# CodeKnight314/Goal-Conditioned-RL-Framework

Measured on AMD Instinct MI355X. Metric: gradient-steps/sec (HER sample + critic+actor update), higher is better.
Workload: dtype f32; 1 GPU; ddpg_pickplace_b256; agent=DDPG, batch_per_gpu=256, buffer_rows=1000000, state_dim=23, action_dim=4, hidden=256, layers=3, k_future=8, gradient_step=40, parallelism=single, hip_graph=True, rng=cpython-mt19937 (host) indices

## Files before the change

goal-conditioned-rl-framework_amd/csrc/agent.hip:

```cpp
#include <hip/hip_runtime.h>

#include <algorithm>
#include <cmath>
#include <cstdlib>
#include <map>
#include <mutex>
#include <random>
#include <string>
#include <vector>

#include "act_bn.h"
#include "dw_adam.h"
#include "gemm_mfma.h"
#include "her_ring.h"
#include "meet.h"
#include "ops.h"
#include "rowchain.h"
#include "sac_heads.h"
#include "xchg_ipc.h"
#include "pop.h"
#include "pbt_host.h"

using namespace gcrl;

// ... 40 lines not shown
  StepCtrl more[kMaxStepsPerCall - 1];
};

}

struct StepPlan { int variant; int tuple_len; };
struct DpSeg { int kind, a, b; float* reduce; long long reduce_n; };

struct gcrl_agent {
  gcrl_agent_config cfg;
  int S = 0, A = 0, H = 0, L = 0, B = 0, C = 0, ldx = 0, Mmax = 0, Apad = 0;
  int Q = 1;
  bool has_target_actor = false, sac = false;
  NetSpec actor, critic;
  hipStream_t stream = nullptr, cap_stream = nullptr;

  float *params = nullptr, *grads = nullptr, *adam_m = nullptr, *adam_v = nullptr;
  long long n_params = 0, n_grads = 0;
  long long off_actor = 0, off_tactor = 0, off_critic = 0, off_tcritic = 0, off_logalpha = 0;
  long long goff_critic = 0, goff_actor = 0, goff_alpha = 0;
  long long critic_stride = 0;
  float *bn_rmean = nullptr, *bn_rvar = nullptr;
  float* alpha_dev = nullptr;

  float* work = nullptr;
  float *sa = nullptr, *nsa = nullptr, *spa = nullptr, *rbuf = nullptr, *dbuf = nullptr;
  long long slot_x = 0, slot_rd = 0;
  float *hTA[2] = {}, *hA = nullptr, *hC = nullptr, *hTC = nullptr, *gC = nullptr, *gA[2] = {};
  float *hC2 = nullptr, *gC2 = nullptr, *bn_part = nullptr;
  float* red_scratch = nullptr;
  float* red_td() const { return red_scratch; }
  float* red_sel() const { return red_scratch + 64LL * ((B + 255) / 256); }
  unsigned int* red_ticket(int i) const { return reinterpret_cast<unsigned int*>(red_scratch + 72LL * ((B + 255) / 256) + 32 * i); }
  float *q = nullptr, *qt = nullptr, *q2 = nullptr, *dq = nullptr, *dq2 = nullptr, *dact = nullptr;
  float *zA = nullptr, *xhatA = nullptr, *invstdA = nullptr, *headA = nullptr, *ghead = nullptr, *dh2 = nullptr;
  float *zN = nullptr, *hN = nullptr, *headN = nullptr, *bn_partN = nullptr;
  float *logp = nullptr, *logp_next = nullptr, *epsbuf = nullptr, *stdbuf = nullptr;
  float *noise_in = nullptr, *eps_next_in = nullptr, *eps_cur_in = nullptr, *norm_partial = nullptr;
  float *w_in = nullptr, *td_abs = nullptr;
  float *act_in = nullptr, *act_tmp[2] = {};
  float *qy = nullptr, *q_row_loss = nullptr, *q_row_td = nullptr;
  float* pi_buf = nullptr;
  float* act_pinned = nullptr;
  char *oa_pinned = nullptr, *oa_dev = nullptr;
  char* act_fl_host = nullptr; char* act_fl_dev = nullptr; unsigned long long act_seq = 0;
  long long oa_calls = 0, oa_launches = 0, oa_copies = 0, oa_syncs = 0;
  size_t oa_bytes = 0;
  bool rowchain = false, wt_dirty = true;
  BnSync bn_sync;
  gcrl_dp* bn_sync_dp = nullptr;
  gcrl_exchange_fn bn_sync_fn = nullptr;
  void* bn_sync_user = nullptr;
  float* bn_sync_buf = nullptr;
  long long bn_sync_cap = 0;
  gcrl_xchg* bn_xchg_h = nullptr;
  int dw_split_c = 1, dw_split_a = 1;
  float *dw_part = nullptr, *dw_tick = nullptr;
  std::vector<long long> dwp_off_c, dwp_off_a, dwt_off_c, dwt_off_a;
  long long dwp_cstride = 0, dwt_cstride = 0, dwp_actor = 0, dwt_actor = 0;
  bool dw_batch_off = false;
  bool bn_slab = false;
  bool slab_on() const { return bn_slab && bn_sync.world <= 1; }
  float* bn_bstat = nullptr;
  float *bn_xchg = nullptr, *bn_bar = nullptr;
  bool bn_split_all = std::getenv("GCRL_NO_SLAB_SPLIT_ALL") == nullptr;
  bool tg_fold_off = std::getenv("GCRL_NO_TG_FOLD") != nullptr;
  bool heads_fold_off = std::getenv("GCRL_NO_HEADS_FOLD") != nullptr;
  const float *hf_eps_next = nullptr, *hf_eps_cur = nullptr;
  int hf_nf = 0;
  int bn_rsplit = 1;
  int bn_slots = 0;
  bool heads_fused_off = false;
  bool red_off = false;
  bool layer_adv_off = false;
  bool bn_fused_tiled = true;
  bool bn_fused = false;
  bool split_k = false;
  bool split_roles = false;
  int n_cus = 0;
  bool rc_merge = false;
  bool rc_merge_k = false;
  bool ddpg_ksplit = false, ddpg_ksplit_can = false;
  bool opt_fuse = false, opt_fuse_can = false;
  long long of_wgs = 0;
  float *of_slots = nullptr, *of_seq = nullptr;
  long long of_stride = 0;
  float* rc_bar = nullptr;
  long long rc_bar_words = 0;
  bool rowtile = false, rowtile_can = false;
  float *rt_xb = nullptr, *rt_qpart = nullptr, *rt_ctr = nullptr, *rt_xid = nullptr;
  long long rt_xb_floats = 0, rt_part_floats = 0;
  long long rt_ctr_words = 0;
  unsigned int *status_host = nullptr, *status_dev = nullptr;
  gcrl_xchg* xchg = nullptr;
  bool xchg_sep_norm = false;
  float xchg_scale() const { return xchg ? 1.0f / (float)gcrl_xchg_world(xchg) : 1.0f; }
  int split_rg[4] = {1, 1, 1, 1};
  int row_rg = 1, row_ldl = 0;
  float *wt = nullptr, *rc_gC = nullptr, *rc_gA = nullptr, *ybuf = nullptr;
  long long wt_net[4] = {};
  long long wt_cstride = 0;
  bool prof = false;
  static constexpr int kProfPairs = 64;
  hipEvent_t prof_a[kProfPairs] = {}, prof_b[kProfPairs] = {};
  unsigned long long* prof_clk = nullptr;
  int prof_used = 0;
  int64_t prof_launches = 0;
  double prof_ms = 0, prof_ticks = 0;
  float *parts_c = nullptr, *parts_a = nullptr;
  int nparts_c = 0, nparts_a = 0, part_off_bn = 0;
  std::vector<int> part_off_c, part_off_a;

  char* upload_dev = nullptr;
  size_t upload_bytes = 0;
  char* upload_pinned[kCtrlSlots] = {};
  hipEvent_t upload_ev[kCtrlSlots] = {};
  int next_upload = 0;
  float *metrics_host = nullptr, *metrics_dev = nullptr;
  int64_t next_ticket = 0;
  int64_t fetched_upto = -1;
  std::vector<int> ticket_len;
  hipEvent_t call_ev[kEventRing] = {};
  int64_t call_last_ticket[kEventRing];
  int64_t calls = 0;

  int64_t t_actor = 0, t_critic = 0, t_alpha = 0;
  double lr_actor = 0, lr_critic = 0;
  uint64_t rng_ctr = 0;
  int pending_variant = 0;
  struct { gcrl_her* her = nullptr; int n = 0; int slot = 0; int next = 0; } deferred;
  int head_batches = 2;
  std::vector<StepPlan> dp_plans;
  std::vector<DpSeg> dp_segs;
  size_t dp_pos = 0;

  std::map<int, hipGraphExec_t> graphs;
  std::map<std::string, std::pair<float*, long long>> names;

  hipStream_t pick(void* s) const {
    if (!s) return stream;
    if (s == GCRL_STREAM_LEGACY) return (hipStream_t) nullptr;
    return (hipStream_t)s;
  }
  CtrlBlock* ctrl() const { return (CtrlBlock*)upload_dev; }
  uint32_t* idx_dev() const { return (uint32_t*)(upload_dev + sizeof(UploadBlock)); }
  const StepCtrl* cur() const { return &ctrl()->cur; }
  const StepCtrl* prev() const { return &ctrl()->prev; }
  const int* slot_ptr() const { return &ctrl()->cur.batch_slot; }
  float* P_actor() const { return params + off_actor; }
  float* P_tactor() const { return params + off_tactor; }
  float* P_critic(int c) const { return params + off_critic + c * critic_stride; }
  float* P_tcritic(int c) const { return params + off_tcritic + c * critic_stride; }
  float* P_logalpha() const { return params + off_logalpha; }
  float* G_actor() const { return grads + goff_actor; }
  float* G_critic(int c) const { return grads + goff_critic + c * critic_stride; }
  float* hC_at(int c, int l) const { return hC + ((long long)c * L + l) * B * H; }
  float* hTC_at(int c, int i) const { return hTC + ((long long)c * 2 + i) * B * H; }
  float* gC_at(int c, int i) const { return gC + ((long long)c * 2 + i) * B * H; }
  float* hC2_at(int l) const { return hC2 + (long long)l * B * H; }
  float* gC2_at(int i) const { return gC2 + (long long)i * B * H; }
  float* hA_at(int l) const { return hA + (long long)l * B * H; }
  int n_actor_critics() const { return (cfg.kind == GCRL_AGENT_DDPG || cfg.kind == GCRL_AGENT_TD3) ? 1 : C; }
};

namespace {

// ... 1047 lines not shown
      {&a->q, (long long)C * B * a->Q}, {&a->qt, (long long)C * B * a->Q}, {&a->q2, (long long)C * B * a->Q}, {&a->dq, (long long)C * B * a->Q},
      {&a->dq2, (long long)C * B * a->Q}, {&a->qy, (long long)B * 64}, {&a->q_row_loss, (long long)C * B}, {&a->q_row_td, B}, {&a->dact, (long long)C * B * a->Apad}, {&a->zA, BH}, {&a->xhatA, L * BH},
      {&a->invstdA, (long long)L * H}, {&a->headA, (long long)B * 2 * a->Apad}, {&a->ghead, (long long)B * 2 * a->Apad},
      {&a->dh2, BH}, {&a->logp, B}, {&a->logp_next, B}, {&a->epsbuf, (long long)B * A}, {&a->stdbuf, (long long)B * A},
      {&a->noise_in, (long long)B * A}, {&a->eps_next_in, (long long)B * A}, {&a->eps_cur_in, (long long)B * A},
      {&a->norm_partial, (long long)kMaxCritics * kNormBlocks}, {&a->act_in, (long long)B * a->ldx},
      {&a->act_tmp[0], BH}, {&a->act_tmp[1], BH},
      {&a->parts_c, (long long)C * a->nparts_c}, {&a->parts_a, (long long)a->nparts_a},
      {&a->hC2, (long long)C * L * BH}, {&a->gC2, 2 * BH}, {&a->bn_part, 2LL * ((B + 15) / 16) * H},
      {&a->rc_gC, (long long)C * L * BH}, {&a->rc_gA, L * BH}, {&a->ybuf, B}, {&a->pi_buf, (long long)B * a->Apad},
      {&a->w_in, B}, {&a->td_abs, B}, {&a->red_scratch, 72LL * ((B + 255) / 256) + 64},
      {&a->bn_bstat, 2LL * 2 * L * H}, {&a->bn_xchg, bn_slab_xchg_floats(H)}, {&a->bn_bar, bn_slab_bar_words(H)}, {&a->zN, BH}, {&a->hN, 2 * BH}, {&a->headN, (long long)B * 2 * a->Apad}, {&a->bn_partN, 2LL * ((B + 15) / 16) * H}};
  {
    const long long per_a = (long long)round_up(S, 4) * H + (long long)(L - 1) * H * H;
    const long long per_c = (long long)a->ldx * H + (long long)(L - 1) * H * H;
    a->wt_cstride = align_up(per_c, 64);
    a->wt_net[0] = 0; a->wt_net[1] = align_up(per_a, 64);
    a->wt_net[2] = 2 * align_up(per_a, 64); a->wt_net[3] = a->wt_net[2] + C * a->wt_cstride;
    wants.push_back({&a->wt, a->wt_net[3] + C * a->wt_cstride});
    a->row_ldl = round_up(std::max(H, a->ldx), 4) + 4;
    a->row_rg = row_rg_of(c.kind, B);
    a->rowchain = (c.kind == GCRL_AGENT_DDPG || c.kind == GCRL_AGENT_TD3 || c.kind == GCRL_AGENT_SAC) && H % 4 == 0 &&
                  c.pipeline_steps >= 2 &&
                  rowchain_lds_bytes(a->row_rg, a->row_ldl, A, H, C) <= 160 * 1024;
    a->split_roles = a->rowchain && c.kind == GCRL_AGENT_SAC && sac_split_roles_rule(C, B, a->row_rg);
    for (int i = 0; i < 4; ++i) a->split_rg[i] = a->row_rg;
    {
      const long long nblk = (B + 4 * a->row_rg - 1) / (4 * a->row_rg);
      a->rc_merge = a->split_roles && !std::getenv("GCRL_NO_RC_MERGE") && !std::getenv("GCRL_SPLIT_RG") &&
                    rowchain_merge_ok(a->row_rg, a->row_ldl, A, H, C, B);
      if (a->rc_merge) { a->rc_bar_words = 2 * nblk * 32; wants.push_back({&a->rc_bar, a->rc_bar_words}); }
    }
    a->split_k = a->rowchain && c.kind == GCRL_AGENT_TD3 && C == 2 && td3_split_k_rule(B, a->row_rg);
    a->rc_merge_k = a->split_k && !meet_device_shared() && !std::getenv("GCRL_NO_RC_MERGE");
    if (a->rc_merge_k && !a->rc_bar_words) {
      const long long nblk = (B + 4 * a->row_rg - 1) / (4 * a->row_rg);
      a->rc_bar_words = 2 * nblk * 32;
      wants.push_back({&a->rc_bar, a->rc_bar_words});
    }
    a->rowtile_can = a->rowchain && c.kind == GCRL_AGENT_DDPG && C == 1 && rowtile_shape_ok(B, H, L, S, A, C);
    a->rowtile = a->rowtile_can && rowtile_enabled() && rowtile_ok(B, H, L, S, A, C);
    if (a->rowtile_can) {
      a->rt_ctr_words = rowtile_ctr_words(B, L);
      a->rt_xb_floats = rowtile_xb_floats(B, H, L); a->rt_part_floats = rowtile_part_floats(B, H);
      wants.push_back({&a->rt_xb, a->rt_xb_floats});
      wants.push_back({&a->rt_qpart, a->rt_part_floats}); wants.push_back({&a->rt_ctr, 2 * a->rt_ctr_words});
      wants.push_back({&a->rt_xid, 3LL * (B / 16) * 32});
    }
    {
      const long long nblk = (B + 4 * a->row_rg - 1) / (4 * a->row_rg);
      static const int per_cu = std::getenv("GCRL_DDPG_KSPLIT_PER_CU") ? std::atoi(std::getenv("GCRL_DDPG_KSPLIT_PER_CU")) : 1;
      a->ddpg_ksplit_can = a->rowchain && c.kind == GCRL_AGENT_DDPG && C == 1 && 3 * nblk <= per_cu * std::max(a->n_cus, 1);
      a->ddpg_ksplit = a->ddpg_ksplit_can && !meet_device_shared() && !std::getenv("GCRL_NO_DDPG_KSPLIT");
      if (a->ddpg_ksplit_can && !a->rc_bar_words) { a->rc_bar_words = 2 * nblk * 32; wants.push_back({&a->rc_bar, a->rc_bar_words}); }
    }
    {
      auto tiles16 = [&](const NetSpec& net, bool* form1) {
        long long t = 0;
        for (const Lin& ln : net.lin) {
          GemmDesc d = bwd_dw(a->grads, 1, a->grads, 1, a->grads, ln, B);
          if (gemm_shape_of(d) != 1) *form1 = false;
          t += (long long)((ln.out + 15) / 16) * ((ln.in + 1 + 15) / 16);
        }
        return t;
      };
      bool form1 = true;
      const long long tc = tiles16(a->critic, &form1), ta = tiles16(a->actor, &form1);
      const long long cap = dw_adam_capacity();
      a->of_stride = align_up(std::max(tc, ta) + 8, 32);
      const bool kind_ok = (c.kind == GCRL_AGENT_DDPG && C == 1) || ((c.kind == GCRL_AGENT_TD3 || c.kind == GCRL_AGENT_SAC) && C == 2);
      a->opt_fuse_can = a->rowchain && kind_ok && L + 1 <= kFusedMaxLayers && form1 && B < 2048 &&
                        std::max(tc, ta) <= 256LL * kFusedMaxSlotsPerThread && 2 * std::max(tc, ta) <= cap;
      a->opt_fuse = a->opt_fuse_can && !meet_device_shared() && !std::getenv("GCRL_NO_OPT_FUSE");
      a->of_wgs = 2 * std::max(tc, ta);
      if (a->opt_fuse_can) {
        wants.push_back({&a->of_slots, (long long)(C + 1) * 2 * a->of_stride * 2});
        wants.push_back({&a->of_seq, (long long)(C + 1) * 32});
      }
    }
    a->head_batches = 3;
    if (c.kind == GCRL_AGENT_DDPG && c.pipeline_steps != 0) a->head_batches = 4;
    if (const char* e = std::getenv("GCRL_HEAD_BATCHES")) a->head_batches = std::max(1, std::min(8, std::atoi(e)));
    a->dw_batch_off = std::getenv("GCRL_NO_DW_BATCH") != nullptr;
    a->bn_fused_tiled = std::getenv("GCRL_NO_BN_TILED_STATS") == nullptr;
    a->layer_adv_off = std::getenv("GCRL_NO_LAYER_ADV") != nullptr;
    a->red_off = std::getenv("GCRL_NO_MB_REDUCE") != nullptr;
    a->heads_fused_off = std::getenv("GCRL_NO_HEADS_FUSED") != nullptr;
    a->bn_fused = std::getenv("GCRL_BN_FUSED") != nullptr;
    if (const char* e = std::getenv("GCRL_SPLIT_RG"))
      for (int i = 0; i < 4 && e[i]; ++i) a->split_rg[i] = e[i] - '0';
  }
  {
    auto tiles_of = [](const Lin& ln) { return (long long)((ln.out + 63) / 64) * ((ln.in + 63) / 64); };
    auto layout = [&](const NetSpec& net, int S, std::vector<long long>& po, std::vector<long long>& to, long long* pn, long long* tn) {
      long long p = 0, t = 0;
      po.clear(); to.clear();
      for (const Lin& ln : net.lin) {
        po.push_back(p); to.push_back(t);
        p += tiles_of(ln) * S * kTiledPartStride;
        t += align_up(tiles_of(ln) * kTicketStride, 64);
      }
      *pn = align_up(p, 64); *tn = t;
    };
    auto pick = [&](long long phase_tiles) {
      int S = 1;
      while (S < 8 && phase_tiles * (S * 2) <= 1280 && B / (16 * S * 2) >= 8) S *= 2;
      return S;
    };
    const bool anyb = std::getenv("GCRL_DW_SPLIT_ANYB") != nullptr;
    const bool on = (B >= 1024 || anyb) && B % 32 == 0 && !std::getenv("GCRL_NO_DW_SPLIT");
    const bool chain_dw = a->rowchain && (c.kind == GCRL_AGENT_DDPG || c.kind == GCRL_AGENT_TD3) && (B >= 2048 || anyb);
    long long tc = 0, ta = 0, big_c = 0;
    for (const Lin& ln : a->critic.lin) { tc += tiles_of(ln); if (ln.out >= 64 && ln.in >= 64) big_c += tiles_of(ln); }
    for (const Lin& ln : a->actor.lin) ta += tiles_of(ln);
    const bool ens = !a->dw_batch_off && L >= 2 && (long long)C * (L - 1) * ((H + 63) / 64) * ((H + 1 + 63) / 64) >= 512;
    if (on && chain_dw) { a->dw_split_c = pick(C * tc); a->dw_split_a = pick(ta); }
    else if (on && ens) a->dw_split_c = pick(C * big_c);
    if (on && a->sac && B >= 2048 && !a->rowchain && !std::getenv("GCRL_NO_DW_SPLIT_ACTOR")) a->dw_split_a = pick((long long)((H + 63) / 64) * ((H + 63) / 64));
    if (const char* e = std::getenv("GCRL_DW_SPLIT")) {
      const int S = std::max(1, std::min(16, std::atoi(e)));
      if (a->dw_split_c > 1) a->dw_split_c = S;
      if (a->dw_split_a > 1) a->dw_split_a = S;
    }
    long long pc = 0, tcn = 0, pa = 0, tan = 0;
    layout(a->critic, a->dw_split_c, a->dwp_off_c, a->dwt_off_c, &pc, &tcn);
    layout(a->actor, a->dw_split_a, a->dwp_off_a, a->dwt_off_a, &pa, &tan);
    a->dwp_cstride = pc; a->dwt_cstride = tcn;
    a->dwp_actor = (long long)C * pc; a->dwt_actor = (long long)C * tcn;
    if (a->dw_split_c > 1 || a->dw_split_a > 1) {
      wants.push_back({&a->dw_part, (long long)C * pc + pa});
      wants.push_back({&a->dw_tick, (long long)C * tcn + tan});
    }
  }
  long long total = 0;
  for (auto& w : wants) total += align_up(w.second, 64);
  TRY(bytes_alloc(&a->work, total));
  long long used = 0;
  for (auto& w : wants) { *w.first = a->work + used; used += align_up(w.second, 64); }
  TRY(rowtile_reset(a));
  TRY(optfuse_reset(a));
  if (a->bn_xchg && a->bn_bar) { TRY(bn_slab_scratch_reset(a->bn_xchg, reinterpret_cast<unsigned int*>(a->bn_bar), H, nullptr)); GCRL_HIP(hipDeviceSynchronize()); }

  a->upload_bytes = sizeof(UploadBlock) + (size_t)kMaxStepsPerCall * B * sizeof(uint32_t);
  GCRL_HIP(hipMalloc((void**)&a->upload_dev, a->upload_bytes));
  GCRL_HIP(hipMemset(a->upload_dev, 0, a->upload_bytes));
  for (int i = 0; i < kCtrlSlots; ++i) {
    GCRL_HIP(hipHostMalloc((void**)&a->upload_pinned[i], a->upload_bytes, hipHostMallocDefault));
    GCRL_HIP(hipEventCreateWithFlags(&a->upload_ev[i], hipEventDisableTiming));
  }
  for (int i = 0; i < kEventRing; ++i) {
    GCRL_HIP(hipEventCreateWithFlags(&a->call_ev[i], hipEventDisableTiming));
    a->call_last_ticket[i] = -1;
  }
  GCRL_HIP(hipHostMalloc((void**)&a->metrics_host, (size_t)kMetricSlots * kMetricFloats * sizeof(float), hipHostMallocDefault));
  std::memset(a->metrics_host, 0, (size_t)kMetricSlots * kMetricFloats * sizeof(float));
  GCRL_HIP(hipMalloc((void**)&a->metrics_dev, (size_t)kMetricSlots * kMetricFloats * sizeof(float)));
  GCRL_HIP(hipMemset(a->metrics_dev, 0, (size_t)kMetricSlots * kMetricFloats * sizeof(float)));
  a->ticket_len.assign(kMetricSlots, 0);

  GCRL_HIP(hipDeviceSynchronize());
  TRY(launch_fill(a->stream, a->dq2, (long long)C * B * a->Q, -1.0f / (float)B));
  TRY(launch_fill(a->stream, a->alpha_dev, 1, 1.0f));
  GCRL_HIP(hipStreamSynchronize(a->stream));

  auto reg = [&](const std::string& k, float* p, long long n) { a->names[k] = {p, n}; };
  reg("actor", a->P_actor(), a->actor.numel);
// ... 889 lines not shown
```

goal-conditioned-rl-framework_amd/csrc/agent_rowchain.inc:

```

struct PipeCtx {
  const StepCtrl* cur;
  const int* slot;
};


RowNet make_rownet(gcrl_agent* a, const NetSpec& n, const float* P, int which, int c = 0) {
  RowNet r;
  std::memset(&r, 0, sizeof(r));
  r.P = P;
  r.Wt = a->wt + a->wt_net[which] + (which >= 2 ? c * a->wt_cstride : 0);
  r.in = n.in_dim; r.jpad0 = round_up(n.in_dim, 4); r.H = n.H; r.L = n.L; r.out = n.out_dim;
  long long off = 0;
  for (int l = 0; l <= n.L; ++l) {
    r.w[l] = n.lin[l].w; r.b[l] = n.lin[l].b;
    if (l < n.L) { r.wt[l] = off; off += (long long)(l == 0 ? r.jpad0 : n.H) * n.H; }
  }
  return r;
}

int rc_rebuild_wt(gcrl_agent* a, hipStream_t st, bool targets_only = false) {
  auto one = [&](const RowNet& r) { return launch_wt_rebuild(st, r, const_cast<float*>(r.Wt)); };
  if (!targets_only && !a->sac) TRY(one(make_rownet(a, a->actor, a->P_actor(), 0)));
  if (a->has_target_actor) TRY(one(make_rownet(a, a->actor, a->P_tactor(), 1)));
// ... 163 lines not shown
  int blk = 0;
  long long pos = 0, off = 0;
  auto flat = [&](long long beg, long long end) {
    if (end <= beg) return;
    AdamSeg& s = ad.seg[ad.n_seg++];
    s.beg = beg; s.dst = 0; s.rows = 1; s.cols = (int)(end - beg); s.tiled = 0; s.pad = 0;
    s.blk0 = blk; s.nblk = (int)((end - beg + 256 * kAdamPerThread - 1) / (256 * kAdamPerThread)); blk += s.nblk;
  };
  for (int l = 0; l < net.L; ++l) {
    const Lin& ln = net.lin[l];
    flat(pos, ln.w);
    AdamSeg& s = ad.seg[ad.n_seg++];
    s.beg = ln.w; s.dst = off; s.rows = ln.out; s.cols = ln.in; s.tiled = 1; s.pad = 0;
    s.blk0 = blk; s.nblk = ((ln.out + kAdamTile - 1) / kAdamTile) * ((ln.in + kAdamTile - 1) / kAdamTile); blk += s.nblk;
    pos = ln.w + (long long)ln.out * ln.in;
    off += (long long)(l == 0 ? round_up(net.in_dim, 4) : net.H) * net.H;
  }
  flat(pos, net.numel);
  ad.seg_blocks = blk;
  if (critic) {
    ad.td_q = a->q; ad.td_y = a->ybuf; ad.td_n = a->B; ad.td_C = a->C;
    ad.td_loss_kind = a->cfg.kind == GCRL_AGENT_TD3 ? LOSS_SMOOTH_L1 : LOSS_MSE;
  }
}

void of_fill_net(gcrl_agent* a, DwAdamNet& n, bool critic, int k, const StepCtrl* cur, bool polyak) {
  const int B = a->B, L = a->L, H = a->H;
  const NetSpec& net = critic ? a->critic : a->actor;
  const long long BH = (long long)B * H;
  std::memset(&n, 0, sizeof(n));
  float* Gp = critic ? a->G_critic(k) : a->G_actor();
  const float* hid = critic ? a->hC + (long long)k * L * BH : a->hA;
  const float* gr = critic ? a->rc_gC + (long long)k * L * BH : a->rc_gA;
  const std::vector<int>& poff = critic ? a->part_off_c : a->part_off_a;
  std::vector<long long> wt_off((size_t)L + 1, -1);
  long long off = 0;
  for (int l = 0; l < L; ++l) { wt_off[l] = off; off += (long long)(l == 0 ? round_up(net.in_dim, 4) : H) * H; }
  int q = 0;
  for (int l = L; l >= 0; --l, ++q) {
    const float* G = l == L ? (critic ? a->dq + (long long)k * B : a->dact) : gr + (long long)l * BH;
    const long long ldg = l == L ? (critic ? 1 : a->Apad) : H;
    GemmDesc dw = bwd_dw(G, ldg, l == 0 ? a->sa : hid + (long long)(l - 1) * BH, l == 0 ? a->ldx : H, Gp, net.lin[l], B);
    if (l == 0) { dw.slot = &cur->batch_slot; dw.b_slot = a->slot_x; }
    n.d[q] = dw;
    n.o.lay[q] = DwAdamLayer{net.lin[l].w, net.lin[l].b, wt_off[l], poff[l] / 4, 0};
  }
  n.o.nl = L + 1;
  n.o.cur = cur;
  n.o.which = critic ? 1 : 0;
  const long long go = critic ? a->goff_critic + (long long)k * a->critic_stride : a->goff_actor;
  n.o.p = critic ? a->P_critic(k) : a->P_actor();
  n.o.m = a->adam_m + go; n.o.v = a->adam_v + go;
  n.o.target = critic ? a->P_tcritic(k) : (polyak ? a->P_tactor() : nullptr);
  n.o.wt = a->wt + a->wt_net[critic ? 2 : 0] + (critic ? (long long)k * a->wt_cstride : 0);
  n.o.wt_target = a->wt + a->wt_net[critic ? 3 : 1] + (critic ? (long long)k * a->wt_cstride : 0);
  n.o.clip = (critic && k == 0 && a->cfg.kind == GCRL_AGENT_TD3) ? -1.f : (float)a->cfg.grad_clip;
  n.o.polyak = polyak ? 1 : 0;
  n.o.metric_index = critic ? MET_CRITIC_GRAD + k : MET_ACTOR_GRAD;
  const int ni = critic ? k : a->C;
  n.o.slots = reinterpret_cast<unsigned long long*>(a->of_slots) + (long long)ni * 2 * a->of_stride;
  n.o.slot_stride = (int)a->of_stride;
  n.o.seq = reinterpret_cast<unsigned int*>(a->of_seq) + ni * 32;
  if (critic) {
    if (k == 0) {
      n.o.td_q = a->q; n.o.td_y = a->ybuf; n.o.td_n = a->B; n.o.td_C = a->C;
      n.o.td_loss_kind = a->cfg.kind == GCRL_AGENT_TD3 ? LOSS_SMOOTH_L1 : LOSS_MSE;
    }
  } else {
    n.o.mean_x = a->q2; n.o.mean_n = a->B; n.o.mean_scale = -1.0f; n.o.mean_index = MET_ACTOR_LOSS;
  }
}

void of_common(gcrl_agent* a, DwAdamArgs& da) {
  std::memset(&da, 0, sizeof(da));
  da.beta2 = (float)kBeta2; da.w1 = (float)(1.0 - kBeta1); da.w2 = (float)(1.0 - kBeta2); da.eps = (float)kAdamEps;
  da.tau = (float)a->cfg.tau; da.one_m_tau = (float)(1.0 - a->cfg.tau);
  da.metrics = a->metrics_dev;
  da.status = a->status_dev;
  static const int first_sleep = std::getenv("GCRL_OF_SLEEP_FIRST") ? std::atoi(std::getenv("GCRL_OF_SLEEP_FIRST")) : 0;
  static const int poll_sleep = std::getenv("GCRL_OF_SLEEP_POLL") ? std::atoi(std::getenv("GCRL_OF_SLEEP_POLL")) : 2;
  static const int gate = std::getenv("GCRL_OF_GATE") ? std::atoi(std::getenv("GCRL_OF_GATE")) : 0;
  static const bool flat = std::getenv("GCRL_OF_FLAT") != nullptr;
  da.poll_first_sleep = first_sleep; da.poll_sleep = poll_sleep; da.poll_gate = gate; da.leaders = flat ? 0 : 1;
}

bool of_phase_critics(const gcrl_agent* a, int variant) {
  return a->opt_fuse && a->cfg.kind != GCRL_AGENT_DDPG && (variant & V_FUSED_NORM) && !(variant & V_XCHG) && !(variant & V_WEIGHTS);
}
bool of_phase_actor(const gcrl_agent* a, int variant) { return of_phase_critics(a, variant) && !a->sac; }
int of_launch_critics(gcrl_agent* a, hipStream_t st, int variant) {
  DwAdamArgs da;
  of_common(a, da);
  for (int k = 0; k < a->C; ++k) of_fill_net(a, da.net[k], true, k, &a->ctrl()->cur_b, (variant & V_POLYAK_C) != 0);
  da.nnets = a->C;
  if ((variant & V_ADV) && !(variant & V_ACTOR)) da.advance = a->ctrl();
  return launch_dw_adam(st, da);
}
int of_launch_actor(gcrl_agent* a, hipStream_t st, int variant) {
  DwAdamArgs da;
  of_common(a, da);
  of_fill_net(a, da.net[0], false, 0, &a->ctrl()->cur_b, a->cfg.kind == GCRL_AGENT_TD3 && (variant & V_POLYAK_A) != 0);
  da.nnets = 1;
  if (variant & V_ADV) da.advance = a->ctrl();
  return launch_dw_adam(st, da);
}

int of_launch_ddpg(gcrl_agent* a, hipStream_t st, int what, bool adv, bool polyak) {
  DwAdamArgs da;
  of_common(a, da);
  int n = 0;
  if (what & 1) of_fill_net(a, da.net[n++], true, 0, &a->ctrl()->cur_b, polyak);
  if (what & 2) of_fill_net(a, da.net[n++], false, 0, what == 3 ? &a->ctrl()->prev_b : &a->ctrl()->cur_b, polyak);
  da.nnets = n;
  if (adv) da.advance = a->ctrl();
#ifdef GCRL_OF_STAMPS
  static unsigned long long* stamps = nullptr;
  static long long launches = 0;
  static const long long at = std::getenv("GCRL_OF_STAMPS_AT") ? std::atoll(std::getenv("GCRL_OF_STAMPS_AT")) : 3000;
  const char* path = std::getenv("GCRL_OF_STAMPS");
  if (path && !stamps) { GCRL_HIP(hipMalloc((void**)&stamps, 2 * 2048 * 8 * sizeof(unsigned long long))); }
  hipStreamCaptureStatus cs = hipStreamCaptureStatusNone;
  (void)hipStreamIsCapturing(st, &cs);
  const bool take = path && what == 3 && cs == hipStreamCaptureStatusNone && launches >= at && launches < at + 8;
  if (what == 3 && cs == hipStreamCaptureStatusNone) ++launches;
  da.stamps = take ? stamps : nullptr;
  if (take) {
    GCRL_HIP(hipMemsetAsync(stamps, 0, 2 * 2048 * 8 * sizeof(unsigned long long), st));
    TRY(launch_dw_adam(st, da));
    GCRL_HIP(hipStreamSynchronize(st));
    std::vector<unsigned long long> h(2 * 2048 * 8);
    GCRL_HIP(hipMemcpy(h.data(), stamps, h.size() * sizeof(unsigned long long), hipMemcpyDeviceToHost));
    FILE* f = std::fopen(path, launches - 1 == at ? "wb" : "ab");
    if (f) { std::fwrite(h.data(), sizeof(unsigned long long), h.size(), f); std::fclose(f); }
    return GCRL_OK;
  }
#endif
  return launch_dw_adam(st, da);
}
```

goal-conditioned-rl-framework_amd/csrc/dw_adam.h:

```cpp
#pragma once
#include "gemm_mfma.h"
#include "ops.h"

namespace gcrl {

struct DwAdamNet {
  DwAdamNetArgs o;
  GemmDesc d[kFusedMaxLayers];
};
struct DwAdamArgs {
  int nnets;
  float beta2, w1, w2, eps, tau, one_m_tau;
  float* metrics;
  CtrlBlock* advance;
  unsigned int* status;
  int leaders;
  int poll_gate;
  int poll_first_sleep, poll_sleep;
#ifdef GCRL_OF_STAMPS
  unsigned long long* stamps;
#endif
  DwAdamNet net[2];
};
int launch_dw_adam(hipStream_t st, DwAdamArgs& a);

}
```

goal-conditioned-rl-framework_amd/csrc/dw_adam.hip:

```cpp
#include "dw_adam.h"

#include <algorithm>

#include "adam_math.h"
#include "meet.h"
#include "pop.h"

namespace gcrl {
namespace {

constexpr unsigned long long kSlotEmpty = ~0ull;
constexpr int kLeaderMinTiles = 64;
static_assert(kFusedMaxLayers == 5, "DwNetHead::tile0 holds the first tiles of problems 1..4");

#ifdef GCRL_OF_STAMPS
#define OF_STAMP(k) of_t[k] = wall_clock64()
#else
#define OF_STAMP(k) do { } while (0)
#endif

template <class T>
__device__ __forceinline__ T load_uniform(const T* p) {
  static_assert(sizeof(T) % 4 == 0, "whole dwords");
  typedef const unsigned int __attribute__((address_space(4))) cu32;
  cu32* q = reinterpret_cast<cu32*>(reinterpret_cast<uintptr_t>(p));
  union { T v; unsigned int w[sizeof(T) / 4]; } u;
#pragma unroll
  for (unsigned i = 0; i < sizeof(T) / 4; ++i) u.w[i] = q[i];
  return u.v;
}

typedef float __attribute__((address_space(1))) gfloat;
typedef unsigned long long __attribute__((address_space(1))) gu64;
typedef unsigned int __attribute__((address_space(1))) gu32;

template <class T>
__device__ __forceinline__ void pin(T& v) {
  static_assert(sizeof(T) % 4 == 0, "whole dwords");
  unsigned int* w = reinterpret_cast<unsigned int*>(&v);
#pragma unroll
  for (unsigned i = 0; i < sizeof(T) / 4; ++i) asm volatile("" : "+s"(w[i]));
}

struct DwProb {
  const float* G; const float* X; float* dW; float* db;
  long long pw, pb, wt_dst;
  int ldg, ldx, out, in, K, tiles_n, slot0, x_slot;
};
struct DwNetHead {
  int ntiles, nl, which, slot_stride;
  int tile0[4];
  const StepCtrl* cur; unsigned int* seq; unsigned long long* slots;
  int polyak, grid_x;
};
struct DwNetPtrs {
  float *p, *m, *v, *target, *wt, *wt_target;
  float clip; int pad;
};
struct DwNetK {
  DwNetHead h;
  DwNetPtrs ptr;
  int metric_index, mean_n;
  const float* mean_x; float mean_scale; int mean_index;
  const float* td_q; const float* td_y; int td_n, td_C, td_loss_kind, pad;
  DwProb prob[kFusedMaxLayers];
};
struct DwAdamK {
  float beta2, w1, w2, eps, tau, one_m_tau;
  int leaders, poll_gate, poll_first_sleep, poll_sleep;
  float* metrics; CtrlBlock* advance; unsigned int* status;
#ifdef GCRL_OF_STAMPS
  unsigned long long* stamps;
#endif
  DwNetK net[2];
};

__global__ __launch_bounds__(256, 5) void dw_adam_kernel(DwAdamK a) {
  const unsigned bx = blockIdx.x, by = blockIdx.y;
#include "dw_adam_body.inc"
}

__global__ __launch_bounds__(256, 5) void dw_adam_pop_kernel(const DwAdamK* __restrict__ tab) {
  const DwAdamK& a = tab[blockIdx.z];
  const unsigned bx = blockIdx.x, by = blockIdx.y;
#include "dw_adam_body.inc"
}

}

long long dw_adam_capacity() { return meet_capacity((const void*)dw_adam_kernel, 256, 0); }

int launch_dw_adam(hipStream_t st, DwAdamArgs& a) {
  GCRL_CHECK_ARG(a.nnets >= 1 && a.nnets <= 2, "dw_adam: %d nets (1 or 2)", a.nnets);
  DwAdamK k;
  std::memset(&k, 0, sizeof(k));
  k.beta2 = a.beta2; k.w1 = a.w1; k.w2 = a.w2; k.eps = a.eps; k.tau = a.tau; k.one_m_tau = a.one_m_tau;
  k.leaders = a.leaders; k.poll_gate = a.poll_gate; k.poll_first_sleep = a.poll_first_sleep; k.poll_sleep = a.poll_sleep;
  k.metrics = a.metrics; k.advance = a.advance; k.status = a.status;
#ifdef GCRL_OF_STAMPS
  k.stamps = a.stamps;
#endif
  int widest = 0;
  for (int i = 0; i < a.nnets; ++i) {
    DwAdamNet& n = a.net[i];
    DwNetK& kn = k.net[i];
    GCRL_CHECK_ARG(n.o.nl >= 1 && n.o.nl <= kFusedMaxLayers && n.o.slots && n.o.seq && n.o.cur, "dw_adam: net %d: %d problems / missing slots", i, n.o.nl);
    int tiles = 0;
    for (int l = 0; l < n.o.nl; ++l) {
      GemmDesc& d = n.d[l];
      GCRL_CHECK_ARG(d.M >= 1 && d.N >= 2 && d.K >= 1 && d.A && d.B && d.C && d.ones_col && d.col_out && !d.bias && d.epi == EPI_NONE && d.mul == MUL_NONE &&
                         !d.bn_part && d.ksplit <= 1 && d.shape_hint == 0 && gemm_shape_of(d) == 1,
                     "dw_adam: net %d problem %d is not a dW | db problem of the k-split 16x16 form", i, l);
      GCRL_CHECK_ARG(d.a_rs == 1 && d.b_cs == 1 && d.c_rs == d.N - 1 && d.a_cs < (1LL << 31) && d.b_rs < (1LL << 31) && d.a_slot == 0 && d.c_slot == 0 &&
                         (!d.slot || (d.slot == &n.o.cur->batch_slot && d.b_slot < (1LL << 31))),
                     "dw_adam: net %d problem %d is not laid out like a dW | db problem", i, l);
      DwProb& p = kn.prob[l];
      p.G = d.A; p.X = d.B; p.dW = d.C; p.db = d.col_out;
      p.pw = n.o.lay[l].pw; p.pb = n.o.lay[l].pb; p.wt_dst = n.o.lay[l].wt_dst;
      p.ldg = (int)d.a_cs; p.ldx = (int)d.b_rs; p.out = d.M; p.in = d.N - 1; p.K = d.K;
      p.tiles_n = (d.N + 15) / 16; p.slot0 = n.o.lay[l].slot0; p.x_slot = d.slot ? (int)d.b_slot : 0;
      if (l >= 1) kn.h.tile0[l - 1] = tiles;
      tiles += ((d.M + 15) / 16) * p.tiles_n;
    }
    n.o.ntiles = tiles;
    GCRL_CHECK_ARG(tiles <= 256 * kFusedMaxSlotsPerThread && tiles + 8 <= n.o.slot_stride, "dw_adam: net %d has %d tiles (slots: %d)", i, tiles, n.o.slot_stride);
    widest = std::max(widest, tiles);
    for (int l = n.o.nl; l < kFusedMaxLayers; ++l) kn.h.tile0[l - 1] = 0x7fffffff;
    kn.h.ntiles = tiles; kn.h.nl = n.o.nl; kn.h.which = n.o.which; kn.h.slot_stride = n.o.slot_stride;
    kn.h.cur = n.o.cur; kn.h.seq = n.o.seq; kn.h.slots = n.o.slots;
    kn.ptr.p = n.o.p; kn.ptr.m = n.o.m; kn.ptr.v = n.o.v; kn.ptr.target = n.o.target; kn.ptr.wt = n.o.wt; kn.ptr.wt_target = n.o.wt_target;
    kn.ptr.clip = n.o.clip; kn.h.polyak = n.o.polyak; kn.metric_index = n.o.metric_index;
    kn.mean_x = n.o.mean_x; kn.mean_n = n.o.mean_n; kn.mean_scale = n.o.mean_scale; kn.mean_index = n.o.mean_index;
    kn.td_q = n.o.td_q; kn.td_y = n.o.td_y; kn.td_n = n.o.td_n; kn.td_C = n.o.td_C; kn.td_loss_kind = n.o.td_loss_kind;
  }
  for (int i = 0; i < a.nnets; ++i) k.net[i].h.grid_x = widest;
  if (PopRec* r = pop_recording())
    return pop_record(r, POP_DW_ADAM, 0, dim3((unsigned)widest, (unsigned)a.nnets), 0, &k, sizeof(k), [k, g = dim3((unsigned)widest, (unsigned)a.nnets)](hipStream_t s) -> int {
      hipLaunchKernelGGL(dw_adam_kernel, g, dim3(256), 0, s, k);
      GCRL_HIP(hipGetLastError());
      return GCRL_OK;
    });
  hipLaunchKernelGGL(dw_adam_kernel, dim3((unsigned)widest, (unsigned)a.nnets), dim3(256), 0, st, k);
  GCRL_HIP(hipGetLastError());
  return GCRL_OK;
}

long long dw_adam_pop_capacity() { return meet_capacity((const void*)dw_adam_pop_kernel, 256, 0); }

int launch_dw_adam_pop(hipStream_t st, const void* tab, int members, dim3 grid) {
  GCRL_CHECK_ARG(members >= 1 && members <= 65535 && grid.y >= 1 && grid.y <= 2 && grid.z == 1, "dw_adam population: bad launch");
  hipLaunchKernelGGL(dw_adam_pop_kernel, dim3(grid.x, grid.y, (unsigned)members), dim3(256), 0, st, static_cast<const DwAdamK*>(tab));
  GCRL_HIP(hipGetLastError());
  return GCRL_OK;
}

}
```

goal-conditioned-rl-framework_amd/csrc/dw_adam_body.inc:

```
#ifdef GCRL_OF_STAMPS
  unsigned long long of_t[5];
#endif
  OF_STAMP(0);
  __shared__ float s_ss[4];
  __shared__ double dred[4];
  __shared__ float s_coef;
  __shared__ float tile_p[16][17], tile_t[16][17];
  const DwNetK& on = a.net[by];
  DwNetHead o = on.h;
  pin(o);
  if ((int)bx >= o.ntiles) return;
  const unsigned long long t_start = wall_clock64();
  int bid = (int)bx;
  {
    const int per = o.ntiles >> 3;
    if (bid < (per << 3)) bid = ((bid + (int)by * o.grid_x) & 7) * per + (bid >> 3);
  }
  const int lane = threadIdx.x & 63;
  const int wave = __builtin_amdgcn_readfirstlane(threadIdx.x >> 6);
  const int li = lane & 15, lg = lane >> 4;
  const int pi = (bid >= o.tile0[0]) + (bid >= o.tile0[1]) + (bid >= o.tile0[2]) + (bid >= o.tile0[3]);
  const int t0 = pi == 0 ? 0 : o.tile0[0] * (pi == 1) + o.tile0[1] * (pi == 2) + o.tile0[2] * (pi == 3) + o.tile0[3] * (pi == 4);
  DwProb pr = on.prob[pi];
  DwNetPtrs ptr = on.ptr;
  StepCtrl c = load_uniform(o.cur);
  unsigned long long sq = load_uniform(reinterpret_cast<const unsigned long long*>(o.seq));
  pin(pr); pin(ptr); pin(c); pin(sq);
  gfloat* const gp = (gfloat*)ptr.p; gfloat* const gm = (gfloat*)ptr.m; gfloat* const gv = (gfloat*)ptr.v; gfloat* const gt = (gfloat*)ptr.target;
  gfloat* const gwt = (gfloat*)ptr.wt; gfloat* const gwtt = (gfloat*)ptr.wt_target;
  gu64* const gslots = (gu64*)o.slots;
  const unsigned int seq = (unsigned int)sq, fault = (unsigned int)(sq >> 32);
  const int t = bid - t0;
  const int tn = t % pr.tiles_n, tm = t / pr.tiles_n;
  const int m0 = tm << 4, n0 = tn << 4;
  const int in = pr.in, out = pr.out;
  struct { long long pw, pb, wt_dst; int slot0; } lay = {pr.pw, pr.pb, pr.wt_dst, pr.slot0};

  const AdamStepScalars sc = adam_scalars(c, o.which);
  const int em = m0 + 4 * lg + wave, en = n0 + li;
  long long my_i = -1;
  if (em < out) {
    if (en < in) my_i = lay.pw + (long long)em * in + en;
    else if (en == in) my_i = lay.pb + em;
  }
  const bool pk = ptr.target && o.polyak;

  GemmDesc d;
  d.A = pr.G; d.a_rs = 1; d.a_cs = pr.ldg;
  d.B = pr.X + (pr.x_slot ? (long long)c.batch_slot * pr.x_slot : 0); d.b_rs = pr.ldx; d.b_cs = 1;
  int one = 1;
  asm volatile("" : "+s"(one));
  d.C = pr.dW; d.c_rs = pr.in; d.col_out = pr.db; d.ones_col = one;
  d.M = pr.out; d.N = pr.in + 1; d.K = pr.K;
  d.bias = nullptr; d.H = nullptr; d.h_rs = 0; d.epi = EPI_NONE; d.mul = MUL_NONE;
  d.slot = nullptr; d.a_slot = d.b_slot = d.c_slot = d.h_slot = 0;
  d.sumsq_out = nullptr; d.bn_part = nullptr;
  d.a_vec = d.b_vec = d.a_rvec = d.b_rvec = 0;
  d.tile0 = 0; d.tiles_n = pr.tiles_n; d.ntiles = 0x7fffffff;
  d.shape_hint = 0; d.ksplit = 0; d.kpart = nullptr; d.kticket = nullptr;
  float x, ss;
  OF_STAMP(1);
  gemm_batch_tile<1, 1, 4>(d, t, x, ss);

#pragma unroll
  for (int off = 32; off > 0; off >>= 1) ss += __shfl_down(ss, off, 64);
  if (lane == 0) s_ss[wave] = ss;
  __syncthreads();
  gu64* mine = gslots + (long long)(seq & 1u) * o.slot_stride;
  if (threadIdx.x == 0 && !(fault && bid == 1)) {
    const double dt = ((double)s_ss[0] + (double)s_ss[1]) + ((double)s_ss[2] + (double)s_ss[3]);
    const int slot = lay.slot0 + t;
    __hip_atomic_store(mine + slot, (unsigned long long)__double_as_longlong(dt), __ATOMIC_RELAXED, __HIP_MEMORY_SCOPE_AGENT);
    gslots[(long long)((seq & 1u) ^ 1u) * o.slot_stride + slot] = kSlotEmpty;
  }
  float pre_p = 0.f, pre_m = 0.f, pre_v = 0.f, pre_t = 0.f;
  if (my_i >= 0) {
    pre_p = gp[my_i]; pre_m = gm[my_i]; pre_v = gv[my_i];
    if (pk) pre_t = gt[my_i];
  }
  OF_STAMP(2);
  float* met = a.metrics + (long long)c.metrics_slot * kMetricFloats;
  if (bid == 0) {
    if (on.mean_x) rider_mean_metric(on.mean_x, on.mean_n, on.mean_scale, met + on.mean_index);
    if (on.td_q) rider_td_metrics(on.td_q, on.td_y, on.td_n, on.td_C, on.td_loss_kind, met);
  }
  {
    const bool lead_mode = a.leaders && o.ntiles >= kLeaderMinTiles;
    const bool sweeper = !lead_mode || bx < 8;
    const int xc = ((int)bx + (int)by * o.grid_x) & 7;
    gu64* res = mine + (o.slot_stride - 8);
    bool ok = true;
    double s = 0.0;
    if (sweeper) {
      unsigned long long w[kFusedMaxSlotsPerThread];
      int spins = 0;
      for (int i = 0; i < a.poll_first_sleep; ++i) __builtin_amdgcn_s_sleep(1);
      for (int i = 0; i < 4096 && (long long)(wall_clock64() - t_start) < (long long)a.poll_gate; ++i) __builtin_amdgcn_s_sleep(2);
#pragma unroll
      for (int u = 0; u < kFusedMaxSlotsPerThread; ++u) {
        const int i = (int)threadIdx.x + 256 * u;
        w[u] = i < o.ntiles ? __hip_atomic_load(mine + i, __ATOMIC_RELAXED, __HIP_MEMORY_SCOPE_AGENT) : 0ull;
      }
      for (;;) {
        bool all = true;
#pragma unroll
        for (int u = 0; u < kFusedMaxSlotsPerThread; ++u) all = all && w[u] != kSlotEmpty;
        if (all) break;
        if (++spins >= kMeetSpinMax) { ok = false; break; }
        for (int i = 0; i < a.poll_sleep; ++i) __builtin_amdgcn_s_sleep(1);
#pragma unroll
        for (int u = 0; u < kFusedMaxSlotsPerThread; ++u)
          if (w[u] == kSlotEmpty) w[u] = __hip_atomic_load(mine + (int)threadIdx.x + 256 * u, __ATOMIC_RELAXED, __HIP_MEMORY_SCOPE_AGENT);
      }
#pragma unroll
      for (int u = 0; u < kFusedMaxSlotsPerThread; ++u)
        if ((int)threadIdx.x + 256 * u < o.ntiles) s += __longlong_as_double((long long)w[u]);
      if (!ok) s = __longlong_as_double(0x7ff8000000000000ll);
      s = wave_sum_d(s);
      if (lane == 0) dred[wave] = s;
      __syncthreads();
      if (threadIdx.x == 0) {
        s = dred[0] + dred[1] + dred[2] + dred[3];
        if (lead_mode) {
          __hip_atomic_store(res + xc, (unsigned long long)__double_as_longlong(s), __ATOMIC_RELAXED, __HIP_MEMORY_SCOPE_AGENT);
          gslots[(long long)((seq & 1u) ^ 1u) * o.slot_stride + (o.slot_stride - 8) + xc] = kSlotEmpty;
        }
      }
    } else if (threadIdx.x == 0) {
      unsigned long long w = __hip_atomic_load(res + xc, __ATOMIC_RELAXED, __HIP_MEMORY_SCOPE_AGENT);
      for (int spins = 0; w == kSlotEmpty; ) {
        if (++spins >= kMeetSpinMax) { ok = false; w = 0x7ff8000000000000ull; break; }
        for (int i = 0; i < a.poll_sleep; ++i) __builtin_amdgcn_s_sleep(1);
        w = __hip_atomic_load(res + xc, __ATOMIC_RELAXED, __HIP_MEMORY_SCOPE_AGENT);
      }
      s = __longlong_as_double((long long)w);
    }
    if (!ok && a.status) __hip_atomic_fetch_or(a.status, (unsigned int)MEET_ERR_DW_ADAM, __ATOMIC_RELAXED, __HIP_MEMORY_SCOPE_SYSTEM);
    if (threadIdx.x == 0) {
      float post;
      s_coef = clip_coef(s, c.grad_scale, ptr.clip, &post);
      if (bid == 0 && a.metrics) met[on.metric_index] = post;
    }
  }
  __syncthreads();
  OF_STAMP(3);
  const float gmul = c.grad_scale * s_coef;
  float p_new = 0.f, t_new = 0.f;
  if (my_i >= 0) {
    const AdamElem e = adam_elem(x, pre_p, pre_m, pre_v, gmul, sc, a.beta2, a.w1, a.w2, a.eps);
    gp[my_i] = e.p; gm[my_i] = e.m; gv[my_i] = e.v;
    p_new = e.p;
    if (pk) { t_new = polyak_elem(a.tau, e.p, a.one_m_tau, pre_t); gt[my_i] = t_new; }
  }
  if (lay.wt_dst >= 0) {
    tile_p[4 * lg + wave][li] = p_new;
    tile_t[4 * lg + wave][li] = t_new;
    __syncthreads();
    const int ty = threadIdx.x >> 4, tx = threadIdx.x & 15;
    const int k = n0 + ty, oo = m0 + tx;
    if (k < in && oo < out) {
      const long long at = lay.wt_dst + (long long)k * out + oo;
      gwt[at] = tile_p[tx][ty];
      if (pk && ptr.wt_target) gwtt[at] = tile_t[tx][ty];
    }
  }
  OF_STAMP(4);
#ifdef GCRL_OF_STAMPS
  if (a.stamps && threadIdx.x == 0)
    for (int k = 0; k < 5; ++k) a.stamps[((long long)by * 2048 + bx) * 8 + k] = of_t[k];
#endif
  if (bid == 0 && threadIdx.x == 0) {
    ((gu32*)o.seq)[1] = 0u;
    ((gu32*)o.seq)[0] = seq + 1u;
    if (by == 0 && a.advance) ctrl_advance(a.advance);
  }
```

Before: 19190 gradient-steps/s.

## Speculatively apply unclipped Adam step before grad-norm reduction completes

The fused dW+Adam kernel now runs the Adam/Polyak update and transposed-weight write assuming a clip coefficient of 1 before waiting on the cross-workgroup gradient-norm reduction. If the reduction then reports clipping, the step is recomputed from the saved pre-update values with the real coefficient. The previous step's clipping status is stored in the seq record and disables speculation for the next step. The aim is to hide the global reduction wait behind the elementwise update, at the cost of redundant work and extra stores whenever clipping is active.

```diff
diff --git a/goal-conditioned-rl-framework_amd/csrc/agent.hip b/goal-conditioned-rl-framework_amd/csrc/agent.hip
--- a/goal-conditioned-rl-framework_amd/csrc/agent.hip
+++ b/goal-conditioned-rl-framework_amd/csrc/agent.hip
@@ -146,6 +146,7 @@
   bool rc_merge_k = false;
   bool ddpg_ksplit = false, ddpg_ksplit_can = false;
   bool opt_fuse = false, opt_fuse_can = false;
+  bool of_no_spec = false;
   long long of_wgs = 0;
   float *of_slots = nullptr, *of_seq = nullptr;
   long long of_stride = 0;
@@ -1359,6 +1360,7 @@
     if (c.kind == GCRL_AGENT_DDPG && c.pipeline_steps != 0) a->head_batches = 4;
     if (const char* e = std::getenv("GCRL_HEAD_BATCHES")) a->head_batches = std::max(1, std::min(8, std::atoi(e)));
     a->dw_batch_off = std::getenv("GCRL_NO_DW_BATCH") != nullptr;
+    a->of_no_spec = std::getenv("GCRL_OF_NO_SPEC") != nullptr;
     a->bn_fused_tiled = std::getenv("GCRL_NO_BN_TILED_STATS") == nullptr;
     a->layer_adv_off = std::getenv("GCRL_NO_LAYER_ADV") != nullptr;
     a->red_off = std::getenv("GCRL_NO_MB_REDUCE") != nullptr;
diff --git a/goal-conditioned-rl-framework_amd/csrc/agent_rowchain.inc b/goal-conditioned-rl-framework_amd/csrc/agent_rowchain.inc
--- a/goal-conditioned-rl-framework_amd/csrc/agent_rowchain.inc
+++ b/goal-conditioned-rl-framework_amd/csrc/agent_rowchain.inc
@@ -269,6 +269,7 @@
   static const int gate = std::getenv("GCRL_OF_GATE") ? std::atoi(std::getenv("GCRL_OF_GATE")) : 0;
   static const bool flat = std::getenv("GCRL_OF_FLAT") != nullptr;
   da.poll_first_sleep = first_sleep; da.poll_sleep = poll_sleep; da.poll_gate = gate; da.leaders = flat ? 0 : 1;
+  da.no_spec = a->of_no_spec ? 1 : 0;
 }
 
 bool of_phase_critics(const gcrl_agent* a, int variant) {
diff --git a/goal-conditioned-rl-framework_amd/csrc/dw_adam.h b/goal-conditioned-rl-framework_amd/csrc/dw_adam.h
--- a/goal-conditioned-rl-framework_amd/csrc/dw_adam.h
+++ b/goal-conditioned-rl-framework_amd/csrc/dw_adam.h
@@ -17,6 +17,7 @@
   int leaders;
   int poll_gate;
   int poll_first_sleep, poll_sleep;
+  int no_spec;
 #ifdef GCRL_OF_STAMPS
   unsigned long long* stamps;
 #endif
diff --git a/goal-conditioned-rl-framework_amd/csrc/dw_adam.hip b/goal-conditioned-rl-framework_amd/csrc/dw_adam.hip
--- a/goal-conditioned-rl-framework_amd/csrc/dw_adam.hip
+++ b/goal-conditioned-rl-framework_amd/csrc/dw_adam.hip
@@ -57,6 +57,9 @@
   float *p, *m, *v, *target, *wt, *wt_target;
   float clip; int pad;
 };
+struct DwSeqRec {
+  unsigned int seq, fault, clipped, pad;
+};
 struct DwNetK {
   DwNetHead h;
   DwNetPtrs ptr;
@@ -67,7 +70,7 @@
 };
 struct DwAdamK {
   float beta2, w1, w2, eps, tau, one_m_tau;
-  int leaders, poll_gate, poll_first_sleep, poll_sleep;
+  int leaders, poll_gate, poll_first_sleep, poll_sleep, no_spec;
   float* metrics; CtrlBlock* advance; unsigned int* status;
 #ifdef GCRL_OF_STAMPS
   unsigned long long* stamps;
@@ -95,7 +98,7 @@
   DwAdamK k;
   std::memset(&k, 0, sizeof(k));
   k.beta2 = a.beta2; k.w1 = a.w1; k.w2 = a.w2; k.eps = a.eps; k.tau = a.tau; k.one_m_tau = a.one_m_tau;
-  k.leaders = a.leaders; k.poll_gate = a.poll_gate; k.poll_first_sleep = a.poll_first_sleep; k.poll_sleep = a.poll_sleep;
+  k.leaders = a.leaders; k.poll_gate = a.poll_gate; k.poll_first_sleep = a.poll_first_sleep; k.poll_sleep = a.poll_sleep; k.no_spec = a.no_spec;
   k.metrics = a.metrics; k.advance = a.advance; k.status = a.status;
 #ifdef GCRL_OF_STAMPS
   k.stamps = a.stamps;
diff --git a/goal-conditioned-rl-framework_amd/csrc/dw_adam_body.inc b/goal-conditioned-rl-framework_amd/csrc/dw_adam_body.inc
--- a/goal-conditioned-rl-framework_amd/csrc/dw_adam_body.inc
+++ b/goal-conditioned-rl-framework_amd/csrc/dw_adam_body.inc
@@ -1,5 +1,5 @@
 #ifdef GCRL_OF_STAMPS
-  unsigned long long of_t[5];
+  unsigned long long of_t[6];
 #endif
   OF_STAMP(0);
   __shared__ float s_ss[4];
@@ -24,12 +24,14 @@
   DwProb pr = on.prob[pi];
   DwNetPtrs ptr = on.ptr;
   StepCtrl c = load_uniform(o.cur);
-  unsigned long long sq = load_uniform(reinterpret_cast<const unsigned long long*>(o.seq));
-  pin(pr); pin(ptr); pin(c); pin(sq);
+  DwSeqRec sq = load_uniform(reinterpret_cast<const DwSeqRec*>(o.seq));
+  struct { float beta2, w1, w2, eps, tau, one_m_tau; int no_spec; } ak = {a.beta2, a.w1, a.w2, a.eps, a.tau, a.one_m_tau, a.no_spec};
+  pin(pr); pin(ptr); pin(c); pin(sq); pin(ak);
   gfloat* const gp = (gfloat*)ptr.p; gfloat* const gm = (gfloat*)ptr.m; gfloat* const gv = (gfloat*)ptr.v; gfloat* const gt = (gfloat*)ptr.target;
   gfloat* const gwt = (gfloat*)ptr.wt; gfloat* const gwtt = (gfloat*)ptr.wt_target;
   gu64* const gslots = (gu64*)o.slots;
-  const unsigned int seq = (unsigned int)sq, fault = (unsigned int)(sq >> 32);
+  const unsigned int seq = sq.seq, fault = sq.fault;
+  const bool spec = !ak.no_spec && !sq.clipped;
   const int t = bid - t0;
   const int tn = t % pr.tiles_n, tm = t / pr.tiles_n;
   const int m0 = tm << 4, n0 = tn << 4;
@@ -84,6 +86,29 @@
     if (on.mean_x) rider_mean_metric(on.mean_x, on.mean_n, on.mean_scale, met + on.mean_index);
     if (on.td_q) rider_td_metrics(on.td_q, on.td_y, on.td_n, on.td_C, on.td_loss_kind, met);
   }
+  auto step = [&](float gmul) {
+    float p_new = 0.f, t_new = 0.f;
+    if (my_i >= 0) {
+      const AdamElem e = adam_elem(x, pre_p, pre_m, pre_v, gmul, sc, ak.beta2, ak.w1, ak.w2, ak.eps);
+      gp[my_i] = e.p; gm[my_i] = e.m; gv[my_i] = e.v;
+      p_new = e.p;
+      if (pk) { t_new = polyak_elem(ak.tau, e.p, ak.one_m_tau, pre_t); gt[my_i] = t_new; }
+    }
+    if (lay.wt_dst >= 0) {
+      tile_p[4 * lg + wave][li] = p_new;
+      tile_t[4 * lg + wave][li] = t_new;
+      __syncthreads();
+      const int ty = threadIdx.x >> 4, tx = threadIdx.x & 15;
+      const int k = n0 + ty, oo = m0 + tx;
+      if (k < in && oo < out) {
+        const long long at = lay.wt_dst + (long long)k * out + oo;
+        gwt[at] = tile_p[tx][ty];
+        if (pk && ptr.wt_target) gwtt[at] = tile_t[tx][ty];
+      }
+    }
+  };
+  if (spec) step(c.grad_scale * 1.0f);
+  OF_STAMP(5);
   {
     const bool lead_mode = a.leaders && o.ntiles >= kLeaderMinTiles;
     const bool sweeper = !lead_mode || bx < 8;
@@ -144,33 +169,15 @@
   }
   __syncthreads();
   OF_STAMP(3);
-  const float gmul = c.grad_scale * s_coef;
-  float p_new = 0.f, t_new = 0.f;
-  if (my_i >= 0) {
-    const AdamElem e = adam_elem(x, pre_p, pre_m, pre_v, gmul, sc, a.beta2, a.w1, a.w2, a.eps);
-    gp[my_i] = e.p; gm[my_i] = e.m; gv[my_i] = e.v;
-    p_new = e.p;
-    if (pk) { t_new = polyak_elem(a.tau, e.p, a.one_m_tau, pre_t); gt[my_i] = t_new; }
-  }
-  if (lay.wt_dst >= 0) {
-    tile_p[4 * lg + wave][li] = p_new;
-    tile_t[4 * lg + wave][li] = t_new;
-    __syncthreads();
-    const int ty = threadIdx.x >> 4, tx = threadIdx.x & 15;
-    const int k = n0 + ty, oo = m0 + tx;
-    if (k < in && oo < out) {
-      const long long at = lay.wt_dst + (long long)k * out + oo;
-      gwt[at] = tile_p[tx][ty];
-      if (pk && ptr.wt_target) gwtt[at] = tile_t[tx][ty];
-    }
-  }
+  if (!spec || s_coef != 1.0f) step(c.grad_scale * s_coef);
   OF_STAMP(4);
 #ifdef GCRL_OF_STAMPS
   if (a.stamps && threadIdx.x == 0)
-    for (int k = 0; k < 5; ++k) a.stamps[((long long)by * 2048 + bx) * 8 + k] = of_t[k];
+    for (int k = 0; k < 6; ++k) a.stamps[((long long)by * 2048 + bx) * 8 + k] = of_t[k];
 #endif
   if (bid == 0 && threadIdx.x == 0) {
     ((gu32*)o.seq)[1] = 0u;
+    ((gu32*)o.seq)[2] = s_coef != 1.0f ? 1u : 0u;
     ((gu32*)o.seq)[0] = seq + 1u;
     if (by == 0 && a.advance) ctrl_advance(a.advance);
   }
```

Measured after the change: 19420 gradient-steps/s, median of 6. 1.2% higher.
